# baler-collaboration/baler

Hardware: AMD Instinct MI355X
Metric: rows/sec (train) + rows/sec (encode), CMS 24-col AE at 1/2/4/8 GPUs (higher is better)
Workload: dtype f32

## Files before the change

### baler_amd/csrc/fused.hip

```cpp
#include "fused.hpp"

#include <cmath>
#include <cstdlib>
#include <type_traits>
#include <utility>

namespace bamd {
namespace {

using v4 = float __attribute__((ext_vector_type(4)));

__host__ __device__ constexpr int tiles(int d) { return (d + 15) / 16; }
__host__ __device__ constexpr int tile_steps(int d, int t) {
    return d - 16 * t >= 16 ? 4 : (d - 16 * t + 3) / 4;
}
__host__ __device__ constexpr int slot_feature(int d, int t, int g, int r) {
    int v = d - 16 * t;
    if (v >= 16) return 16 * t + 4 * g + r;
    return 4 * r + g < v ? 16 * t + 4 * r + g : -1;
}

constexpr int kQS = 68;
constexpr int kRowsPerWG = 64;

#ifndef BAMD_SPLIT
#define BAMD_SPLIT 2
#endif
constexpr int kSplit = BAMD_SPLIT;

template <int F, int Z> struct Net {
    static constexpr int L = 8;
    __host__ __device__ static constexpr int dim(int i) {
        return i == 0 ? F : i == 1 ? 200 : i == 2 ? 100 : i == 3 ? 50 : i == 4 ? Z : i == 5 ? 50 : i == 6 ? 100 : i == 7 ? 200 : F;
    }
    __host__ __device__ static constexpr bool act(int l) { return !(l == 3 || l == 7); }
    __host__ __device__ static constexpr int wcount(int l) { return tiles(dim(l)) * tiles(dim(l + 1)) * 64; }
    __host__ __device__ static constexpr int wf_off(int l) { int s = 0; for (int j = 0; j < l; ++j) s += wcount(j); return s; }
    __host__ __device__ static constexpr int wb_off(int l) { int s = wf_off(L); for (int j = L - 1; j > l; --j) s += wcount(j); return s; }
    __host__ __device__ static constexpr int bf_off(int l) { int s = wb_off(0); for (int j = 0; j < l; ++j) s += tiles(dim(j + 1)) * 4; return s; }
    __host__ __device__ static constexpr int e_off() { return (bf_off(L) + 63) / 64 * 64; }
    __host__ __device__ static constexpr int ef_off(int l) { return e_off() + wf_off(l); }
    __host__ __device__ static constexpr int eb_off(int l) { int s = e_off() + wf_off(kSplit - 1); for (int j = kSplit - 1; j > l; --j) s += wcount(j); return s; }
    __host__ __device__ static constexpr int l4_off() { return eb_off(0) + 16 * 64; }
    __host__ __device__ static constexpr int l4_gemm_k(int g) { return g < 8 ? dim(g) : dim(15 - g + 1); }
    __host__ __device__ static constexpr int l4_gemm_n(int g) { return g < 8 ? dim(g + 1) : dim(15 - g); }
    __host__ __device__ static constexpr int l4_groups(int g) { return (l4_gemm_n(g) + 63) / 64; }
    __host__ __device__ static constexpr int l4_ks(int g) { return (l4_gemm_k(g) + 3) / 4; }
    __host__ __device__ static constexpr int l4_frag_off(int g) { int s = 0; for (int j = 0; j < g; ++j) s += l4_gemm_n(j) * l4_ks(j); return s; }
    __host__ __device__ static constexpr int l4_frags() { return F <= 32 ? l4_frag_off(15) : 0; }
    __host__ __device__ static constexpr int packed_f4() { return l4_off() + l4_frags() + 16 * 64; }
    __host__ __device__ static constexpr int dw_tiles(int l) { return tiles(dim(l + 1)) * tiles(dim(l) + 1); }
    __host__ __device__ static constexpr int slab_off(int l) { int s = 0; for (int j = 0; j < l; ++j) s += dw_tiles(j); return s; }
    __host__ __device__ static constexpr int slab_f4() { return slab_off(L) * 64 + 4; }
    __host__ __device__ static constexpr int w_off(int l) { int s = 0; for (int j = 0; j < l; ++j) s += dim(j + 1) * dim(j) + dim(j + 1); return s; }
    __host__ __device__ static constexpr int b_off(int l) { return w_off(l) + dim(l + 1) * dim(l); }
    __host__ __device__ static constexpr int nparams() { return w_off(L); }
};

__device__ __forceinline__ v4 mfma(float a, float b, v4 c) { return __builtin_amdgcn_mfma_f32_16x16x4f32(a, b, c, 0, 0, 0); }

typedef unsigned int u4 __attribute__((ext_vector_type(4)));
struct WStream {
    __amdgpu_buffer_rsrc_t rsrc;
    int voff;
};
__device__ __forceinline__ WStream make_stream(const v4 *base, int bytes, int lane) {
    WStream ws;
    ws.rsrc = __builtin_amdgcn_make_buffer_rsrc((void *)base, 0, bytes, 0x00020000);
    ws.voff = lane * 16;
    return ws;
}
__device__ __forceinline__ v4 frag(const WStream &ws, int idx) {
    return __builtin_bit_cast(v4, __builtin_amdgcn_raw_buffer_load_b128(ws.rsrc, ws.voff, idx * 1024, 0));
}
__device__ __forceinline__ v4 frag_rt(const WStream &ws, int idx) {
    return __builtin_bit_cast(v4, __builtin_amdgcn_raw_buffer_load_b128(ws.rsrc, ws.voff, idx * 1024, 0));
}
#ifndef BAMD_RING
#define BAMD_RING 8
#endif
constexpr int kRing = BAMD_RING;
#ifndef BAMD_CHAIN_WAYS
#define BAMD_CHAIN_WAYS 2
#endif
struct Ring { v4 slot[kRing]; };

__host__ __device__ constexpr int pad_total(int t) { return (t + kRing - 1) / kRing * kRing; }

template <int TOTAL>
__device__ __forceinline__ void ring_prime(Ring &ring, const WStream &ws) {
    static_assert(TOTAL >= kRing, "stream shorter than the ring");
#pragma unroll
    for (int i = 0; i < kRing; ++i) ring.slot[i] = frag(ws, i);
}
template <int TOTAL>
__device__ __forceinline__ void ring_tail(Ring &ring, const WStream &ws) {
#pragma unroll
    for (int G = TOTAL; G < pad_total(TOTAL); ++G)
        ring.slot[G % kRing] = frag(ws, (G + kRing) % pad_total(TOTAL));
    __builtin_amdgcn_sched_barrier(0);
}

template <int KD, int NT, int BASE, int TOTAL>
__device__ __forceinline__ void chain_gemm(const v4 (&in)[tiles(KD)], v4 (&out)[NT], Ring &ring, const WStream &ws) {
    constexpr int NF = tiles(KD) * NT;
    constexpr int W = BAMD_CHAIN_WAYS;
#pragma unroll
    for (int f = 0; f < NF; f += W) {
#pragma unroll
        for (int r = 0; r < 4; ++r)
#pragma unroll
            for (int j = 0; j < W; ++j)
                if (f + j < NF && r < tile_steps(KD, (f + j) / NT))
                    out[(f + j) % NT] = mfma(ring.slot[(BASE + f + j) % kRing][r], in[(f + j) / NT][r], out[(f + j) % NT]);
#pragma unroll
        for (int j = 0; j < W; ++j)
            if (f + j < NF)
                ring.slot[(BASE + f + j) % kRing] = frag(ws, (BASE + f + j + kRing) % pad_total(TOTAL));
        __builtin_amdgcn_sched_barrier(0);
    }
}

template <int KD, int NT, int BASE, int TOTAL>
__device__ __forceinline__ void chain_gemm2(const v4 (&in0)[tiles(KD)], const v4 (&in1)[tiles(KD)], v4 (&out0)[NT], v4 (&out1)[NT],
                                            Ring &ring, const WStream &ws) {
    constexpr int NF = tiles(KD) * NT;
#pragma unroll
    for (int f = 0; f < NF; ++f) {
#pragma unroll
        for (int r = 0; r < 4; ++r)
            if (r < tile_steps(KD, f / NT)) {
                out0[f % NT] = mfma(ring.slot[(BASE + f) % kRing][r], in0[f / NT][r], out0[f % NT]);
                out1[f % NT] = mfma(ring.slot[(BASE + f) % kRing][r], in1[f / NT][r], out1[f % NT]);
            }
        ring.slot[(BASE + f) % kRing] = frag(ws, (BASE + f + kRing) % pad_total(TOTAL));
        __builtin_amdgcn_sched_barrier(0);
    }
}

template <int NT> __device__ __forceinline__ void init_bias(v4 (&out)[NT], const v4 *bias_lds, int lane) {
#pragma unroll
    for (int t = 0; t < NT; ++t) out[t] = bias_lds[t * 4 + (lane >> 4)];
}
template <int NT> __device__ __forceinline__ void zero_tiles(v4 (&out)[NT]) {
#pragma unroll
    for (int t = 0; t < NT; ++t) out[t] = (v4){0.f, 0.f, 0.f, 0.f};
}
template <int NT> __device__ __forceinline__ void lrelu(v4 (&a)[NT]) {
    typedef float v2f __attribute__((ext_vector_type(2)));
    v2f k2 = (v2f){0.01f, 0.01f};
    asm volatile("" : "+v"(k2));
    const v4 kk = (v4){k2[0], k2[1], k2[0], k2[1]};
#pragma unroll
    for (int t = 0; t < NT; ++t) {
        v4 m = a[t] * kk;
        asm("" : "+v"(m));
#pragma unroll
        for (int r = 0; r < 4; ++r) a[t][r] = __builtin_elementwise_maximum(a[t][r], m[r]);
    }
}
template <int NT> __device__ __forceinline__ void lrelu_bwd(v4 (&d)[NT], const v4 (&y)[NT]) {
#pragma unroll
    for (int t = 0; t < NT; ++t) {
        v4 sl;
#pragma unroll
        for (int r = 0; r < 4; ++r) sl[r] = y[t][r] > 0.f ? 1.0f : 0.01f;
        d[t] = d[t] * sl;
    }
}

template <class N, class S, int l>
__device__ __forceinline__ void fwd_layer(const v4 (&in)[tiles(N::dim(l))], v4 (&out)[tiles(N::dim(l + 1))],
                                          Ring &ring, const WStream &ws, const v4 *bias_lds, int lane) {
    init_bias(out, bias_lds + (N::bf_off(l) - N::bf_off(0)), lane);
    chain_gemm<N::dim(l), tiles(N::dim(l + 1)), S::fwd_base(l), S::total>(in, out, ring, ws);
    if (N::act(l)) lrelu(out);
}
template <class N, class S, int l>
__device__ __forceinline__ void fwd_layer2(const v4 (&in0)[tiles(N::dim(l))], const v4 (&in1)[tiles(N::dim(l))],
                                           v4 (&out0)[tiles(N::dim(l + 1))], v4 (&out1)[tiles(N::dim(l + 1))], Ring &ring,
                                           const WStream &ws, const v4 *bias_lds, int lane) {
    init_bias(out0, bias_lds + (N::bf_off(l) - N::bf_off(0)), lane);
#pragma unroll
    for (int t = 0; t < tiles(N::dim(l + 1)); ++t) out1[t] = out0[t];
    chain_gemm2<N::dim(l), tiles(N::dim(l + 1)), S::fwd_base(l), S::total>(in0, in1, out0, out1, ring, ws);
    if (N::act(l)) { lrelu(out0); lrelu(out1); }
}
template <class N, class S, int l>
__device__ __forceinline__ void bwd_layer(const v4 (&dz)[tiles(N::dim(l + 1))], v4 (&dx)[tiles(N::dim(l))],
                                          Ring &ring, const WStream &ws) {
    zero_tiles(dx);
    chain_gemm<N::dim(l + 1), tiles(N::dim(l)), S::bwd_base(l), S::total>(dz, dx, ring, ws);
}

template <class N> struct StreamEncode {
    static constexpr int fwd_base(int l) { return N::wf_off(l) / 64; }
    static constexpr int total = N::wf_off(4) / 64;
    static constexpr int start_f4 = 0;
};
template <class N> struct StreamDecode {
    static constexpr int fwd_base(int l) { return (N::wf_off(l) - N::wf_off(4)) / 64; }
    static constexpr int total = (N::wf_off(8) - N::wf_off(4)) / 64;
    static constexpr int start_f4 = N::wf_off(4);
};
template <class N> struct StreamForward {
    static constexpr int fwd_base(int l) { return N::wf_off(l) / 64; }
    static constexpr int total = N::wf_off(8) / 64;
    static constexpr int start_f4 = 0;
};
template <class N> struct StreamTrainDec {
    static constexpr int fwd_base(int l) { return N::wf_off(l) / 64; }
    static constexpr int bwd_base(int l) { return N::wb_off(l) / 64; }
    static constexpr int total = N::wb_off(kSplit - 1) / 64;
    static constexpr int start_f4 = 0;
};
template <class N> struct StreamTrainEnc {
    static constexpr int fwd_base(int l) { return (N::ef_off(l) - N::e_off()) / 64; }
    static constexpr int bwd_base(int l) { return (N::eb_off(l) - N::e_off()) / 64; }
    static constexpr int total = (N::eb_off(0) - N::e_off()) / 64;
    static constexpr int start_f4 = N::e_off();
};

template <class N> struct StreamWideEnc {
    static constexpr int fwd_base(int l) { return (N::wf_off(l) - N::wf_off(1)) / 64; }
    static constexpr int total = (N::wf_off(4) - N::wf_off(1)) / 64;
    static constexpr int start_f4 = N::wf_off(1);
// ... 1823 lines not shown
        load_w(wr[1], xa[1], xb[1], 1);
        load_w(wr[2], xa[2], xb[2], 2);
        for (int t0 = 0; t0 < KTF; t0 += 8) {
            load_w(wr[3], xa[3], xb[3], t0 + 3);
            tile_out(wr[0], xa[0], xb[0], t0, std::integral_constant<int, 0>());
            __builtin_amdgcn_sched_barrier(0);
            load_w(wr[0], xa[0], xb[0], t0 + 4);
            tile_out(wr[1], xa[1], xb[1], t0 + 1, std::integral_constant<int, 1>());
            __builtin_amdgcn_sched_barrier(0);
            load_w(wr[1], xa[1], xb[1], t0 + 5);
            tile_out(wr[2], xa[2], xb[2], t0 + 2, std::integral_constant<int, 2>());
            __builtin_amdgcn_sched_barrier(0);
            load_w(wr[2], xa[2], xb[2], t0 + 6);
            tile_out(wr[3], xa[3], xb[3], t0 + 3, std::integral_constant<int, 3>());
            __builtin_amdgcn_sched_barrier(0);
            load_w(wr[3], xa[3], xb[3], t0 + 7);
            tile_out(wr[0], xa[0], xb[0], t0 + 4, std::integral_constant<int, 4>());
            __builtin_amdgcn_sched_barrier(0);
            load_w(wr[0], xa[0], xb[0], t0 + 8);
            tile_out(wr[1], xa[1], xb[1], t0 + 5, std::integral_constant<int, 5>());
            __builtin_amdgcn_sched_barrier(0);
            load_w(wr[1], xa[1], xb[1], t0 + 9);
            tile_out(wr[2], xa[2], xb[2], t0 + 6, std::integral_constant<int, 6>());
            __builtin_amdgcn_sched_barrier(0);
            load_w(wr[2], xa[2], xb[2], t0 + 10);
            tile_out(wr[3], xa[3], xb[3], t0 + 7, std::integral_constant<int, 7>());
            __builtin_amdgcn_sched_barrier(0);
        }
        if (F % 16 != 0) {
            constexpr int t = KT - 1;
            v4 o0 = bias7[t * 4 + g], o1 = o0;
#pragma unroll
            for (int c = 0; c < 7; ++c) {
                const bf8 w = frag_bf(w7, t * 7 + c);
                o0 = mfma_bf(w, qa[c], o0);
                o1 = mfma_bf(w, qb[c], o1);
            }
            const v4 d0 = o0 - wide_x_chunk<F>(x, 0, rr0, t, g), d1 = o1 - wide_x_chunk<F>(x, 0, rr1, t, g);
            if (v0) {
                lacc += (double)(d0[0] * d0[0] + d0[1] * d0[1]) + (double)(d0[2] * d0[2] + d0[3] * d0[3]);
                if constexpr (DZ16) wide_store_tile_bf16<F>(d0 * gscale, dz8h, r0, t, g); else wide_store_tile<F>(d0 * gscale, dz8, 0, r0, t, g);
            }
            if (v1) {
                lacc += (double)(d1[0] * d1[0] + d1[1] * d1[1]) + (double)(d1[2] * d1[2] + d1[3] * d1[3]);
                if constexpr (DZ16) wide_store_tile_bf16<F>(d1 * gscale, dz8h, r1, t, g); else wide_store_tile<F>(d1 * gscale, dz8, 0, r1, t, g);
            }
        }
    }
    const double wsum = block_sum_tree(lacc, sh);
    if (threadIdx.x == 0) loss_part[blockIdx.x] = wsum;
}

template <int F, int Z, bool DZ16>
__global__ void __launch_bounds__(256) wide_bf16_train_bwd_kernel(const v4 *packed, const v4 *w7tb, const void *__restrict__ dz7, int64_t n,
                                                                  const float *__restrict__ y1, const float *__restrict__ y2,
                                                                  const float *__restrict__ y3, const float *__restrict__ y5,
                                                                  const float *__restrict__ y6, const float *__restrict__ y7,
                                                                  float *__restrict__ dz0, float *__restrict__ dz1, float *__restrict__ dz2,
                                                                  float *__restrict__ dz3, float *__restrict__ dz4, float *__restrict__ dz5,
                                                                  float *__restrict__ dz6, const float *__restrict__ dz_latent) {
    using N = Net<F, Z>;
    using S = StreamWideMidBwd<N>;
    constexpr int KBT = (F + 31) / 32;
    __shared__ __attribute__((aligned(16))) v4 wst[2][13][64];
    const int lane = threadIdx.x & 63, wave = __builtin_amdgcn_readfirstlane(threadIdx.x >> 6), g = lane >> 4;
    const int64_t ngroup = (n + 127) / 128;
    WStream ws = make_stream(packed + S::start_f4, (N::packed_f4() - S::start_f4) * 16, lane);
    WStream w7 = make_stream(w7tb, KBT * 13 * 1024, lane);
    for (int64_t grp = blockIdx.x; grp < ngroup; grp += gridDim.x) {
        const int64_t r0 = (grp * 4 + wave) * 32 + (lane & 15), r1 = r0 + 16;
        const bool v0 = r0 < n, v1 = r1 < n;
        constexpr int es = DZ16 ? 2 : 4;
        const __amdgpu_buffer_rsrc_t xrs = __builtin_amdgcn_make_buffer_rsrc((void *)((const char *)dz7 + (size_t)(grp * 128) * F * es), 0,
                                                                             0x7fffffff, 0x00020000);
        const int lr0 = wave * 32 + (lane & 15);
        const int xo0 = ((v0 ? lr0 : 0) * F + 8 * g) * es, xo1 = ((v1 ? lr0 + 16 : 0) * F + 8 * g) * es;
        asm volatile("" : "+v"(ws.voff), "+v"(w7.voff));
        v4 d6a[13], d6b[13];
        zero_tiles(d6a);
        zero_tiles(d6b);
        wide_in_product_bf16<F, DZ16>(d6a, d6b, wst, w7, xrs, xo0, xo1, wave, lane, g);
        auto narrow = [&](v4 (&d6)[13], int64_t row, bool valid) {
            const int64_t rrow = valid ? row : 0;
            Ring ring;
            ring_prime<S::total>(ring, ws);
            {
                v4 a[13];
                load_act<200>(a, y7, rrow, g);
                lrelu_bwd(d6, a);
            }
            store_rows<200>(d6, dz6, 0, row, valid, lane, nullptr, nullptr);
            v4 d5[7], d4[4], d3[tiles(Z)], d2[4], d1[7], d0[13];
            bwd_layer<N, S, 6>(d6, d5, ring, ws);
            { v4 a[7]; load_act<100>(a, y6, rrow, g); lrelu_bwd(d5, a); }
            store_rows<100>(d5, dz5, 0, row, valid, lane, nullptr, nullptr);
            bwd_layer<N, S, 5>(d5, d4, ring, ws);
            { v4 a[4]; load_act<50>(a, y5, rrow, g); lrelu_bwd(d4, a); }
            store_rows<50>(d4, dz4, 0, row, valid, lane, nullptr, nullptr);
            bwd_layer<N, S, 4>(d4, d3, ring, ws);
            if (dz_latent) {
                v4 e[tiles(Z)];
                load_act<Z>(e, dz_latent, rrow, g);
#pragma unroll
                for (int t = 0; t < tiles(Z); ++t) d3[t] += e[t];
            }
            store_rows<Z>(d3, dz3, 0, row, valid, lane, nullptr, nullptr);
            bwd_layer<N, S, 3>(d3, d2, ring, ws);
            { v4 a[4]; load_act<50>(a, y3, rrow, g); lrelu_bwd(d2, a); }
            store_rows<50>(d2, dz2, 0, row, valid, lane, nullptr, nullptr);
            bwd_layer<N, S, 2>(d2, d1, ring, ws);
            { v4 a[7]; load_act<100>(a, y2, rrow, g); lrelu_bwd(d1, a); }
            store_rows<100>(d1, dz1, 0, row, valid, lane, nullptr, nullptr);
            bwd_layer<N, S, 1>(d1, d0, ring, ws);
            { v4 a[13]; load_act<200>(a, y1, rrow, g); lrelu_bwd(d0, a); }
            store_rows<200>(d0, dz0, 0, row, valid, lane, nullptr, nullptr);
        };
        narrow(d6a, r0, v0);
        narrow(d6b, r1, v1);
    }
}

template <int NT>
__device__ __forceinline__ void q_write(float *__restrict__ q, const v4 (&a)[NT], int lane, int wave) {
    typedef float __attribute__((address_space(3))) *lds_f;
    const int col = 16 * wave + (lane & 15), g = lane >> 4;
#pragma unroll
    for (int r = 0; r < 4; ++r) {
        lds_f p = (lds_f)q + ((4 * g + r) * kQS + col);
        asm volatile("" : "+v"(p));
#pragma unroll
        for (int t = 0; t < NT; ++t) p[t * 16 * kQS] = a[t][r];
    }
}
template <int D>
__device__ __forceinline__ void q_write_x(float *__restrict__ q, const v4 (&a)[tiles(D)], int lane, int wave) {
    static_assert(D % 16 != 0, "ones slot lives in the partial last tile");
    constexpr int T = tiles(D) - 1, V = D - 16 * T;
    constexpr int R1 = V / 4, G1 = V % 4;
    typedef float __attribute__((address_space(3))) *lds_f;
    const int col = 16 * wave + (lane & 15), g = lane >> 4;
#pragma unroll
    for (int r = 0; r < 4; ++r) {
        lds_f p = (lds_f)q + ((4 * g + r) * kQS + col);
        asm volatile("" : "+v"(p));
#pragma unroll
        for (int t = 0; t < tiles(D); ++t) {
            float v = a[t][r];
            if (t == T && r == R1 && g == G1) v = 1.0f;
            p[t * 16 * kQS] = v;
        }
    }
}

template <class N, int l> struct DW {
    static constexpr int NT = tiles(N::dim(l + 1)), KT = tiles(N::dim(l) + 1), TOT = NT * KT, T = (TOT + 3) / 4;
    static constexpr int rows_x = 16 * KT, rows_dz = 16 * NT;
};

template <class N, int l>
__device__ __forceinline__ void dw_phase(const float *__restrict__ qdz, const float *__restrict__ qx,
                                         v4 (&acc)[DW<N, l>::T], int lane, int wave) {
    using D = DW<N, l>;
    constexpr int NP = (D::T + 1) / 2, U = 4 * NP;
    const int g = lane >> 4, i = lane & 15;
    typedef const float __attribute__((address_space(3))) *lds_cf;
    typedef const v4 __attribute__((address_space(3))) *lds_cv4;
    const lds_cf la = (lds_cf)qdz + (i * kQS + 4 * g), lb = (lds_cf)qx + (i * kQS + 4 * g);
    const lds_cf la_w = la + wave * (16 * kQS);
    v4 fa[2][2], fb[2][2];
    auto lds_frags = [&](int u, v4 (&a)[2], v4 (&b)[2]) {
#pragma unroll
        for (int h = 0; h < 2; ++h) {
            const int it = 2 * (u >> 2) + h;
            if (it < D::T) {
                const int c = (4 * it) % D::NT, k0 = (4 * it) / D::NT;
                if (c + 3 < D::NT && 4 * it + 3 < D::TOT) {
                    a[h] = *(lds_cv4)(la_w + c * (16 * kQS) + 16 * (u & 3));
                    b[h] = *(lds_cv4)(lb + k0 * (16 * kQS) + 16 * (u & 3));
                } else {
                    int idx = wave + 4 * it;
                    idx = idx < D::TOT ? idx : D::TOT - 1;
                    const int kt = idx / D::NT, nt = idx - kt * D::NT;
                    a[h] = *(lds_cv4)(la + nt * (16 * kQS) + 16 * (u & 3));
                    b[h] = *(lds_cv4)(lb + kt * (16 * kQS) + 16 * (u & 3));
                }
            }
        }
    };
    lds_frags(0, fa[0], fb[0]);
#pragma unroll
    for (int u = 0; u < U; ++u) {
        if (u + 1 < U) lds_frags(u + 1, fa[(u + 1) & 1], fb[(u + 1) & 1]);
        __builtin_amdgcn_sched_barrier(0);
        const int it0 = 2 * (u >> 2), it1 = it0 + 1;
#pragma unroll
        for (int r = 0; r < 4; ++r) {
            acc[it0] = mfma(fa[u & 1][0][r], fb[u & 1][0][r], acc[it0]);
            if (it1 < D::T) acc[it1] = mfma(fa[u & 1][1][r], fb[u & 1][1][r], acc[it1]);
        }
        __builtin_amdgcn_sched_barrier(0);
    }
}

template <class N, int l>
__device__ __forceinline__ void dw_flush(v4 *__restrict__ slab, const v4 (&acc)[DW<N, l>::T], int lane, int wave) {
#pragma unroll
    for (int it = 0; it < DW<N, l>::T; ++it) {
        const int idx = wave + 4 * it;
        if (idx < DW<N, l>::TOT) slab[(int64_t)(N::slab_off(l) + idx) * gridDim.x * 64 + lane] = acc[it];
    }
}

constexpr int kImgB = 320;
template <class N> constexpr int img_a_rows();
template <class N> constexpr bool train_bias_in_lds() {
    return (size_t)(img_a_rows<N>() + kImgB) * kQS * sizeof(float) + (size_t)(N::bf_off(8) - N::bf_off(0)) * 16 <= 160 * 1024;
}
template <class N> constexpr int img_a_rows() {
    int m = 240;
    const int need[] = {DW<N, 7>::rows_x + DW<N, 7>::rows_dz, DW<N, 5>::rows_x + DW<N, 5>::rows_dz, DW<N, 2>::rows_x + DW<N, 2>::rows_dz,
                        DW<N, 0>::rows_x + DW<N, 0>::rows_dz};
    for (int v : need) m = v > m ? v : m;
    return m;
}

template <int F, int Z, bool RT = false>
__global__ void __launch_bounds__(256) train_dec_kernel(const v4 *packed, const void *__restrict__ xin, int in_f64,
                                                        int64_t n, const double *__restrict__ feats, v4 *__restrict__ slabs,
                                                        v4 *__restrict__ dz_out, int fr, int zr) {
    using N = Net<F, Z>;
    using S = StreamTrainDec<N>;
    constexpr int kImgA = img_a_rows<N>();
    static_assert(DW<N, 7>::rows_x + DW<N, 7>::rows_dz <= kImgA && DW<N, 6>::rows_x + DW<N, 6>::rows_dz <= kImgB &&
                  DW<N, 5>::rows_x + DW<N, 5>::rows_dz <= kImgA && DW<N, 4>::rows_x + DW<N, 4>::rows_dz <= kImgB, "image buffers");
    extern __shared__ __attribute__((aligned(16))) float lds[];
    float *imgA = lds, *imgB = lds + kImgA * kQS;
    const v4 *bias_lds = packed + N::bf_off(0);
    if constexpr (train_bias_in_lds<N>()) {
        v4 *stage = (v4 *)(lds + (kImgA + kImgB) * kQS);
        stage_bias<N>(stage, packed);
        bias_lds = stage;
    }
    int lane = threadIdx.x & 63, wave = __builtin_amdgcn_readfirstlane(threadIdx.x >> 6);
    v4 *slab = slabs + (int64_t)blockIdx.x * 64;
    const int64_t ngroups = (n + kRowsPerWG - 1) / kRowsPerWG;
    WStream ws = make_stream(packed + S::start_f4, (N::packed_f4() - S::start_f4) * 16, threadIdx.x & 63);
    double lacc = 0.0;
    v4 g7[DW<N, 7>::T], g6[DW<N, 6>::T], g5[DW<N, 5>::T], g4[DW<N, 4>::T];
    zero_tiles(g7); zero_tiles(g6); zero_tiles(g5); zero_tiles(g4);
#if BAMD_SPLIT == 2
    v4 g3[DW<N, 3>::T], g2[DW<N, 2>::T];
    zero_tiles(g3); zero_tiles(g2);
#endif
    Ring ring;
    ring_prime<S::total>(ring, ws);
    v4 a0n[tiles(F)];
    {
        const int64_t row0 = (int64_t)blockIdx.x * kRowsPerWG + 16 * wave + (lane & 15);
        load_rows<F, RT>(a0n, xin, in_f64, row0, row0 < n, lane, feats, fr);
    }
    for (int64_t grp = blockIdx.x; grp < ngroups; grp += gridDim.x) {
        asm volatile("" : "+v"(ws.voff), "+s"(wave), "+v"(lane));
        const int64_t row = grp * kRowsPerWG + 16 * wave + (lane & 15);
        const bool valid = row < n;
        const int64_t row_next = row + (int64_t)gridDim.x * kRowsPerWG;
        const bool valid_next = row_next < n;
        RawRows<F> xraw;
        v4 a4[tiles(Z)], a5[4], a6[7], a7[13], d8[tiles(F)];
#if BAMD_SPLIT == 2
        v4 a2[7], a3[4];
#endif
        {
#if BAMD_SPLIT == 2
            v4 a0[tiles(F)], a1[13];
#else
            v4 a0[tiles(F)], a1[13], a2[7], a3[4];
#endif
#pragma unroll
            for (int t = 0; t < tiles(F); ++t) a0[t] = a0n[t];
            fwd_layer<N, S, 0>(a0, a1, ring, ws, bias_lds, lane);
            fwd_layer<N, S, 1>(a1, a2, ring, ws, bias_lds, lane);
            fwd_layer<N, S, 2>(a2, a3, ring, ws, bias_lds, lane);
            fwd_layer<N, S, 3>(a3, a4, ring, ws, bias_lds, lane);
            fwd_layer<N, S, 4>(a4, a5, ring, ws, bias_lds, lane);
            fwd_layer<N, S, 5>(a5, a6, ring, ws, bias_lds, lane);
            fwd_layer<N, S, 6>(a6, a7, ring, ws, bias_lds, lane);
            fwd_layer<N, S, 7>(a7, d8, ring, ws, bias_lds, lane);
#pragma unroll
            for (int t = 0; t < tiles(F); ++t)
#pragma unroll
                for (int r = 0; r < 4; ++r) {
                    float d = d8[t][r] - a0[t][r];
                    const bool live = valid && slot_feature(F, t, lane >> 4, r) >= 0;
                    if (live) lacc += (double)d * (double)d;
                    d8[t][r] = live ? d * (2.0f / (float)(RT ? fr : F)) : 0.f;
                }
        }
        v4 d7[13], d6[7], d5[4], d4[tiles(Z)];
        q_write_x<200>(imgA, a7, lane, wave); q_write(imgA + DW<N, 7>::rows_x * kQS, d8, lane, wave);
        bwd_layer<N, S, 7>(d8, d7, ring, ws); lrelu_bwd(d7, a7);
        __syncthreads();
        dw_phase<N, 7>(imgA + DW<N, 7>::rows_x * kQS, imgA, g7, lane, wave);

        q_write_x<100>(imgB, a6, lane, wave); q_write(imgB + DW<N, 6>::rows_x * kQS, d7, lane, wave);
        bwd_layer<N, S, 6>(d7, d6, ring, ws); lrelu_bwd(d6, a6);
        __syncthreads();
        load_rows_issue<F, RT>(xraw, xin, in_f64, row_next, valid_next, lane, fr);
        dw_phase<N, 6>(imgB + DW<N, 6>::rows_x * kQS, imgB, g6, lane, wave);
        load_rows_finish<F, RT>(a0n, xraw, valid_next, lane, feats, fr);

        q_write_x<50>(imgA, a5, lane, wave); q_write(imgA + DW<N, 5>::rows_x * kQS, d6, lane, wave);
        bwd_layer<N, S, 5>(d6, d5, ring, ws); lrelu_bwd(d5, a5);
        __syncthreads();
        dw_phase<N, 5>(imgA + DW<N, 5>::rows_x * kQS, imgA, g5, lane, wave);

        q_write_x<Z>(imgB, a4, lane, wave); q_write(imgB + DW<N, 4>::rows_x * kQS, d5, lane, wave);
        bwd_layer<N, S, 4>(d5, d4, ring, ws);
#if BAMD_SPLIT == 4
        if (valid) dz_out[row * 4 + (lane >> 4)] = d4[0];
#endif
        __syncthreads();
        dw_phase<N, 4>(imgB + DW<N, 4>::rows_x * kQS, imgB, g4, lane, wave);
#if BAMD_SPLIT == 2
        v4 d3[4], d2[7];
        q_write_x<50>(imgA, a3, lane, wave); q_write(imgA + DW<N, 3>::rows_x * kQS, d4, lane, wave);
        bwd_layer<N, S, 3>(d4, d3, ring, ws); lrelu_bwd(d3, a3);
        __syncthreads();
        dw_phase<N, 3>(imgA + DW<N, 3>::rows_x * kQS, imgA, g3, lane, wave);

        q_write_x<100>(imgB, a2, lane, wave); q_write(imgB + DW<N, 2>::rows_x * kQS, d3, lane, wave);
        bwd_layer<N, S, 2>(d3, d2, ring, ws); lrelu_bwd(d2, a2);
#pragma unroll
        for (int t = 0; t < 7; ++t) dz_out[((row >> 4) * 7 + t) * 64 + lane] = d2[t];
        __syncthreads();
        dw_phase<N, 2>(imgB + DW<N, 2>::rows_x * kQS, imgB, g2, lane, wave);
#endif
        ring_tail<S::total>(ring, ws);
    }
    dw_flush<N, 7>(slab, g7, lane, wave); dw_flush<N, 6>(slab, g6, lane, wave);
    dw_flush<N, 5>(slab, g5, lane, wave); dw_flush<N, 4>(slab, g4, lane, wave);
#if BAMD_SPLIT == 2
    dw_flush<N, 3>(slab, g3, lane, wave); dw_flush<N, 2>(slab, g2, lane, wave);
#endif
    __syncthreads();
    const double wsum = block_sum_tree(lacc, (double *)lds);
    if (threadIdx.x == 0) ((double *)(slabs + (int64_t)N::slab_off(N::L) * gridDim.x * 64))[blockIdx.x] = wsum;
}

#if BAMD_SPLIT == 2
template <int F, int Z, bool RT = false>
__global__ void __launch_bounds__(256) train_enc_kernel(const v4 *packed, const void *__restrict__ xin, int in_f64,
                                                        int64_t n, const double *__restrict__ feats, v4 *__restrict__ slabs,
                                                        const v4 *__restrict__ dz_in, int fr, int zr) {
    using N = Net<F, Z>;
    using S = StreamTrainEnc<N>;
    constexpr int kImgA = img_a_rows<N>();
    static_assert(DW<N, 1>::rows_x + DW<N, 1>::rows_dz <= kImgB && DW<N, 0>::rows_x + DW<N, 0>::rows_dz <= kImgA, "image buffers");
    extern __shared__ __attribute__((aligned(16))) float lds[];
    float *imgA = lds, *imgB = lds + kImgA * kQS;
    const v4 *bias_lds = packed + N::bf_off(0);
    if constexpr (train_bias_in_lds<N>()) {
        v4 *stage = (v4 *)(lds + (kImgA + kImgB) * kQS);
        stage_bias<N>(stage, packed);
// ... 1901 lines not shown
```

Measured before the change: 298.9 million.

## Deal weight-gradient tiles to waves as 2x2 blocks for LDS fragment reuse

Replaces the round-robin assignment of weight-gradient output tiles to waves with a compile-time deal that groups tiles into 2x2, 2x1 and 1x2 blocks. Within a block each A and B fragment loaded from LDS feeds two MFMAs, cutting LDS reads per MFMA. Per-wave tile indices are chosen with a packed-constant pick, and the flush writes each tile to its dealt slab index. Separately, the weight-stream fragment load moves the low bits of the index into the voffset register, keeping the immediate offset aligned. This adds heavy template metaprogramming and may raise register pressure.

```diff
diff --git a/baler_amd/csrc/fused.hip b/baler_amd/csrc/fused.hip
--- a/baler_amd/csrc/fused.hip
+++ b/baler_amd/csrc/fused.hip
@@ -71,7 +71,7 @@
     return ws;
 }
 __device__ __forceinline__ v4 frag(const WStream &ws, int idx) {
-    return __builtin_bit_cast(v4, __builtin_amdgcn_raw_buffer_load_b128(ws.rsrc, ws.voff, idx * 1024, 0));
+    return __builtin_bit_cast(v4, __builtin_amdgcn_raw_buffer_load_b128(ws.rsrc, ws.voff + (idx & 3) * 1024, (idx & ~3) * 1024, 0));
 }
 __device__ __forceinline__ v4 frag_rt(const WStream &ws, int idx) {
     return __builtin_bit_cast(v4, __builtin_amdgcn_raw_buffer_load_b128(ws.rsrc, ws.voff, idx * 1024, 0));
@@ -2201,63 +2201,150 @@
     }
 }
 
+template <int NT_, int KT_> struct DwDeal {
+    static constexpr int NT = NT_, KT = KT_, TOT = NT * KT, T = (TOT + 3) / 4;
+    int q = 0, h = 0, v = 0, s = 0;
+    int nt[4][T] = {}, kt[4][T] = {};
+    bool live[4][T] = {};
+    constexpr int units() const { return q + h + v + (s + 1) / 2; }
+};
+struct DwUnit { int base, n, na, nb, fa[4], fb[4], sa[2], sb[2]; };
+template <int NT, int KT> constexpr DwUnit dw_unit(const DwDeal<NT, KT> &d, int u) {
+    if (u < d.q) return {4 * u, 4, 2, 2, {0, 0, 1, 1}, {0, 1, 0, 1}, {4 * u, 4 * u + 2}, {4 * u, 4 * u + 1}};
+    int b = 4 * d.q;
+    u -= d.q;
+    if (u < d.h) return {b + 2 * u, 2, 1, 2, {0, 0, 0, 0}, {0, 1, 0, 0}, {b + 2 * u, 0}, {b + 2 * u, b + 2 * u + 1}};
+    b += 2 * d.h;
+    u -= d.h;
+    if (u < d.v) return {b + 2 * u, 2, 2, 1, {0, 1, 0, 0}, {0, 0, 0, 0}, {b + 2 * u, b + 2 * u + 1}, {b + 2 * u, 0}};
+    b += 2 * d.v;
+    u -= d.v;
+    if (2 * u + 1 < d.s) return {b + 2 * u, 2, 2, 2, {0, 1, 0, 0}, {0, 1, 0, 0}, {b + 2 * u, b + 2 * u + 1}, {b + 2 * u, b + 2 * u + 1}};
+    return {b + 2 * u, 1, 1, 1, {0, 0, 0, 0}, {0, 0, 0, 0}, {b + 2 * u, 0}, {b + 2 * u, 0}};
+}
+template <int NT, int KT> constexpr DwDeal<NT, KT> dw_deal() {
+    DwDeal<NT, KT> d;
+    constexpr int M = NT * KT + 8;
+    int qn[M] = {}, qk[M] = {}, hn[M] = {}, hk[M] = {}, vn[M] = {}, vk[M] = {}, sn[M] = {}, sk[M] = {};
+    int nq = 0, nh = 0, nv = 0, ns = 0;
+    for (int a = 0; a < KT / 2; ++a)
+        for (int b = 0; b < NT / 2; ++b) { qn[nq] = 2 * b; qk[nq++] = 2 * a; }
+    if (NT % 2) for (int a = 0; a < KT / 2; ++a) { hn[nh] = NT - 1; hk[nh++] = 2 * a; }
+    if (KT % 2) for (int b = 0; b < NT / 2; ++b) { vn[nv] = 2 * b; vk[nv++] = KT - 1; }
+    if (NT % 2 && KT % 2) { sn[ns] = NT - 1; sk[ns++] = KT - 1; }
+    d.q = nq / 4;
+    for (int i = 4 * d.q; i < nq; ++i)
+        for (int j = 0; j < 2; ++j) { hn[nh] = qn[i] + j; hk[nh++] = qk[i]; }
+    d.h = nh / 4;
+    for (int i = 4 * d.h; i < nh; ++i)
+        for (int j = 0; j < 2; ++j) { sn[ns] = hn[i]; sk[ns++] = hk[i] + j; }
+    d.v = nv / 4;
+    for (int i = 4 * d.v; i < nv; ++i)
+        for (int j = 0; j < 2; ++j) { sn[ns] = vn[i] + j; sk[ns++] = vk[i]; }
+    d.s = (ns + 3) / 4;
+    for (int w = 0; w < 4; ++w) {
+        int at = 0;
+        for (int u = 0; u < d.q; ++u)
+            for (int j = 0; j < 4; ++j, ++at) { d.nt[w][at] = qn[4 * u + w] + j / 2; d.kt[w][at] = qk[4 * u + w] + j % 2; d.live[w][at] = true; }
+        for (int u = 0; u < d.h; ++u)
+            for (int j = 0; j < 2; ++j, ++at) { d.nt[w][at] = hn[4 * u + w]; d.kt[w][at] = hk[4 * u + w] + j; d.live[w][at] = true; }
+        for (int u = 0; u < d.v; ++u)
+            for (int j = 0; j < 2; ++j, ++at) { d.nt[w][at] = vn[4 * u + w] + j; d.kt[w][at] = vk[4 * u + w]; d.live[w][at] = true; }
+        for (int u = 0; u < d.s; ++u, ++at) {
+            const int i = 4 * u + w, c = i < ns ? i : ns - 1;
+            d.nt[w][at] = sn[c]; d.kt[w][at] = sk[c]; d.live[w][at] = i < ns;
+        }
+    }
+    return d;
+}
+template <int NT, int KT> constexpr bool dw_deal_ok(const DwDeal<NT, KT> &d) {
+    if (4 * d.q + 2 * d.h + 2 * d.v + d.s != d.T) return false;
+    int seen[NT * KT] = {};
+    for (int w = 0; w < 4; ++w)
+        for (int a = 0; a < d.T; ++a) {
+            if (d.nt[w][a] < 0 || d.nt[w][a] >= NT || d.kt[w][a] < 0 || d.kt[w][a] >= KT) return false;
+            if (d.live[w][a]) seen[d.kt[w][a] * NT + d.nt[w][a]]++;
+        }
+    for (int t = 0; t < NT * KT; ++t)
+        if (seen[t] != 1) return false;
+    return true;
+}
+
 template <class N, int l> struct DW {
     static constexpr int NT = tiles(N::dim(l + 1)), KT = tiles(N::dim(l) + 1), TOT = NT * KT, T = (TOT + 3) / 4;
     static constexpr int rows_x = 16 * KT, rows_dz = 16 * NT;
+    static constexpr DwDeal<NT, KT> deal = dw_deal<NT, KT>();
+    static_assert(dw_deal_ok(deal), "weight-gradient tile deal");
+    static_assert(TOT <= 256 && NT <= 15 && KT <= 15, "dw_pick packs a wave's value into 8 bits");
 };
+
+template <class Fn, int... I> __device__ __forceinline__ void static_for(Fn &&fn, std::integer_sequence<int, I...>) {
+    (fn(std::integral_constant<int, I>{}), ...);
+}
+template <int C0, int C1, int C2, int C3> __device__ __forceinline__ int dw_pick(int wave) {
+    if constexpr (C0 == C1 && C1 == C2 && C2 == C3) return C0;
+    else if constexpr (C1 - C0 == C2 - C1 && C2 - C1 == C3 - C2) return C0 + wave * (C1 - C0);
+    else return (int)(((unsigned)C0 | (unsigned)C1 << 8 | (unsigned)C2 << 16 | (unsigned)C3 << 24) >> (8 * wave) & 0xffu);
+}
 
 template <class N, int l>
 __device__ __forceinline__ void dw_phase(const float *__restrict__ qdz, const float *__restrict__ qx,
                                          v4 (&acc)[DW<N, l>::T], int lane, int wave) {
     using D = DW<N, l>;
-    constexpr int NP = (D::T + 1) / 2, U = 4 * NP;
+    constexpr int U = 4 * D::deal.units();
     const int g = lane >> 4, i = lane & 15;
     typedef const float __attribute__((address_space(3))) *lds_cf;
     typedef const v4 __attribute__((address_space(3))) *lds_cv4;
     const lds_cf la = (lds_cf)qdz + (i * kQS + 4 * g), lb = (lds_cf)qx + (i * kQS + 4 * g);
-    const lds_cf la_w = la + wave * (16 * kQS);
     v4 fa[2][2], fb[2][2];
-    auto lds_frags = [&](int u, v4 (&a)[2], v4 (&b)[2]) {
-#pragma unroll
-        for (int h = 0; h < 2; ++h) {
-            const int it = 2 * (u >> 2) + h;
-            if (it < D::T) {
-                const int c = (4 * it) % D::NT, k0 = (4 * it) / D::NT;
-                if (c + 3 < D::NT && 4 * it + 3 < D::TOT) {
-                    a[h] = *(lds_cv4)(la_w + c * (16 * kQS) + 16 * (u & 3));
-                    b[h] = *(lds_cv4)(lb + k0 * (16 * kQS) + 16 * (u & 3));
-                } else {
-                    int idx = wave + 4 * it;
-                    idx = idx < D::TOT ? idx : D::TOT - 1;
-                    const int kt = idx / D::NT, nt = idx - kt * D::NT;
-                    a[h] = *(lds_cv4)(la + nt * (16 * kQS) + 16 * (u & 3));
-                    b[h] = *(lds_cv4)(lb + kt * (16 * kQS) + 16 * (u & 3));
-                }
-            }
+    auto lds_frags = [&](auto uc, v4 (&a)[2], v4 (&b)[2]) {
+        constexpr int u = decltype(uc)::value;
+        constexpr DwUnit un = dw_unit(D::deal, u >> 2);
+        constexpr int a0 = un.sa[0], a1 = un.sa[1], b0 = un.sb[0], b1 = un.sb[1];
+        const lds_cf pa = la + dw_pick<D::deal.nt[0][a0], D::deal.nt[1][a0], D::deal.nt[2][a0], D::deal.nt[3][a0]>(wave) * (16 * kQS);
+        const lds_cf pb = lb + dw_pick<D::deal.kt[0][b0], D::deal.kt[1][b0], D::deal.kt[2][b0], D::deal.kt[3][b0]>(wave) * (16 * kQS);
+        a[0] = *(lds_cv4)(pa + 16 * (u & 3));
+        b[0] = *(lds_cv4)(pb + 16 * (u & 3));
+        if constexpr (un.na == 2) {
+            if constexpr (un.n == 2 && un.nb == 2)
+                a[1] = *(lds_cv4)(la + dw_pick<D::deal.nt[0][a1], D::deal.nt[1][a1], D::deal.nt[2][a1], D::deal.nt[3][a1]>(wave) * (16 * kQS) +
+                                  16 * (u & 3));
+            else a[1] = *(lds_cv4)(pa + 16 * kQS + 16 * (u & 3));
+        }
+        if constexpr (un.nb == 2) {
+            if constexpr (un.n == 2 && un.na == 2)
+                b[1] = *(lds_cv4)(lb + dw_pick<D::deal.kt[0][b1], D::deal.kt[1][b1], D::deal.kt[2][b1], D::deal.kt[3][b1]>(wave) * (16 * kQS) +
+                                  16 * (u & 3));
+            else b[1] = *(lds_cv4)(pb + 16 * kQS + 16 * (u & 3));
         }
     };
-    lds_frags(0, fa[0], fb[0]);
-#pragma unroll
-    for (int u = 0; u < U; ++u) {
-        if (u + 1 < U) lds_frags(u + 1, fa[(u + 1) & 1], fb[(u + 1) & 1]);
+    auto step = [&](auto uc) {
+        constexpr int u = decltype(uc)::value;
+        constexpr DwUnit un = dw_unit(D::deal, u >> 2);
+        if constexpr (u + 1 < U) lds_frags(std::integral_constant<int, u + 1>{}, fa[(u + 1) & 1], fb[(u + 1) & 1]);
         __builtin_amdgcn_sched_barrier(0);
-        const int it0 = 2 * (u >> 2), it1 = it0 + 1;
-#pragma unroll
-        for (int r = 0; r < 4; ++r) {
-            acc[it0] = mfma(fa[u & 1][0][r], fb[u & 1][0][r], acc[it0]);
-            if (it1 < D::T) acc[it1] = mfma(fa[u & 1][1][r], fb[u & 1][1][r], acc[it1]);
-        }
+#pragma unroll
+        for (int r = 0; r < 4; ++r)
+#pragma unroll
+            for (int j = 0; j < un.n; ++j)
+                acc[un.base + j] = mfma(fa[u & 1][un.fa[j]][r], fb[u & 1][un.fb[j]][r], acc[un.base + j]);
         __builtin_amdgcn_sched_barrier(0);
-    }
+    };
+    lds_frags(std::integral_constant<int, 0>{}, fa[0], fb[0]);
+    static_for(step, std::make_integer_sequence<int, U>{});
 }
 
 template <class N, int l>
 __device__ __forceinline__ void dw_flush(v4 *__restrict__ slab, const v4 (&acc)[DW<N, l>::T], int lane, int wave) {
-#pragma unroll
-    for (int it = 0; it < DW<N, l>::T; ++it) {
-        const int idx = wave + 4 * it;
-        if (idx < DW<N, l>::TOT) slab[(int64_t)(N::slab_off(l) + idx) * gridDim.x * 64 + lane] = acc[it];
-    }
+    using D = DW<N, l>;
+    auto store = [&](auto ac) {
+        constexpr int A = decltype(ac)::value;
+        const int idx = dw_pick<D::deal.kt[0][A] * D::NT + D::deal.nt[0][A], D::deal.kt[1][A] * D::NT + D::deal.nt[1][A],
+                                D::deal.kt[2][A] * D::NT + D::deal.nt[2][A], D::deal.kt[3][A] * D::NT + D::deal.nt[3][A]>(wave);
+        const bool live = dw_pick<D::deal.live[0][A], D::deal.live[1][A], D::deal.live[2][A], D::deal.live[3][A]>(wave) != 0;
+        if (live) slab[(int64_t)(N::slab_off(l) + idx) * gridDim.x * 64 + lane] = acc[A];
+    };
+    static_for(store, std::make_integer_sequence<int, D::T>{});
 }
 
 constexpr int kImgB = 320;
```

Result: no change. 298.7 million (-0.1%).
